# alexcoca/DistributedKernelShap

Measured on NVIDIA H100. Metric: instances explained/sec (bg=100, nsamples=2048) at 1/2/4/8 H100 vs ray CPU, higher is better.
Workload: dtype f32 sigmoid/accumulate, f64 link + WLS

## Files before the change

### distributedkernelshap_b200/csrc/dks.cu

```cuda
#include <algorithm>
#include <cmath>
#include <cstdarg>
#include <cstdio>
#include <cstring>
#include <memory>

#include "dks_kernels.cuh"
#include "dks_tc.cuh"
#include "dks_shared.cuh"
#include "dks_fused.cuh"
#include "dks_l1.cuh"
#include "dks_mixture.cuh"
#include "dks_multi.cuh"
#include "dks_wide.cuh"
#include "dks_sampler.cuh"
#include "dks_instance_wide.cuh"
#include "dks_trees.cuh"
#include "dks_encode.cuh"
#include "dks_kmach.cuh"
#include "dks_mlp.cuh"
#include "dks_knn.cuh"
#include "dks_ensemble.cuh"

namespace {
// ... 467 lines not shown
            m->own_X = ctx->own_X; m->own_D = ctx->own_D; m->own_bg = ctx->own_bg;
            m->own_goff = ctx->own_goff; m->own_gcols = ctx->own_gcols;
            const size_t msm = own_kernel(m->head.family).smem(m, p.S_cap);
            const dks::EnsAcc mea{ctx->d_ens_ey, ctx->h_ens_pi[k], k == 0 ? 1 : 0};
            TRY(on_member(ctx, m, [&] { return launch_own_kernel(m, false, p, msm, st, mea); }));
        }
        const size_t tsm = dks::ens::tail_smem_bytes(p.S_cap, ctx->C);
        auto kern = l1 ? dks::ens::explain_ensemble_tail_kernel<true> : dks::ens::explain_ensemble_tail_kernel<false>;
        CUDA_TRY(cudaFuncSetAttribute(kern, cudaFuncAttributeMaxDynamicSharedMemorySize, (int)tsm));
        kern<<<persistent_grid(ctx, tsm, 1024, 8, ctx->cur_n), dks::ens::THREADS, tsm, st>>>(p, q, ctx->d_ens_ey);
        break;
    }
    }
    ctx->launches += 1;
    return DKS_OK;
}

template <bool STAGE, bool MAPS>
decltype(&dks::prep_kernel<STAGE, MAPS>) prep_kernel_for(bool mixture, int R) {
    if (mixture) return dks::prep_kernel<STAGE, MAPS, true>;
    return R == 1 ? dks::prep_kernel<STAGE, MAPS, false, 1> : dks::prep_kernel<STAGE, MAPS, false, 8>;
}

int launch_prepare(dks_ctx* ctx, const double* X_dev, int n) {
    const int G = ctx->G;
    const HeadDesc& h = ctx->head;
    TRY(ensure_workspace(ctx, n));
    CUDA_TRY(cudaMemsetAsync(ctx->d_status, 0, sizeof(int) * (4 + G + 1), ctx->stream));
    if (!ctx->capturing) ctx->last_was_graph = false;
    CUDA_TRY(record_ev(ctx, 0));
    int ipb = 256 / G;
    if (ipb < 1) ipb = 1;
    const bool maps = ctx->cm.hdr != nullptr;
    const size_t maps_doubles = maps ? (size_t)ctx->cm.n_keys + ctx->cm.n_vals : 0;
    const bool stage = dks::prep_smem_bytes(true, ipb, G, ctx->R, ctx->D, maps_doubles) <= (size_t)96 * 1024;
    const size_t psm = dks::prep_smem_bytes(stage, ipb, G, ctx->R, ctx->D, maps_doubles);
    const bool own = h.own();
    const int R = own ? 1 : ctx->R;
    auto kern = stage ? (maps ? prep_kernel_for<true, true>(h.mixture(), R) : prep_kernel_for<true, false>(h.mixture(), R))
                      : (maps ? prep_kernel_for<false, true>(h.mixture(), R) : prep_kernel_for<false, false>(h.mixture(), R));
    double* xt = !own && (h.xt_any || (G <= 128 && ctx->plan_mode == 0)) ? ctx->d_XT.get() : nullptr;
    if (psm > 48 * 1024) CUDA_TRY(cudaFuncSetAttribute(kern, cudaFuncAttributeMaxDynamicSharedMemorySize, (int)psm));
    const bool enc = own && ctx->enc.E > 0;
    if (enc) TRY(grow(ctx, ctx->d_Xenc, (size_t)n * ctx->enc.E));
    ctx->own_X = enc ? ctx->d_Xenc : X_dev;
    ctx->own_D = enc ? ctx->enc.E : ctx->D;
    ctx->own_bg = enc ? ctx->d_bg_enc : ctx->d_bg;
    ctx->own_goff = enc ? ctx->d_egoff : ctx->d_goff;
    ctx->own_gcols = enc ? ctx->d_egcols : ctx->d_gcols;
    kern<<<cdiv(n, ipb), 256, psm, ctx->stream>>>(
        X_dev, ctx->d_W, ctx->d_b, ctx->d_bg, ctx->d_goff, ctx->d_gcols, ctx->d_colmin, ctx->d_colmax, ctx->d_colnan,
        ctx->d_linkfnull, n, ctx->N, ctx->D, G, R, own ? 1 : ctx->C, own ? DKS_ACT_IDENTITY : ctx->act, own ? 1.0 : ctx->kappa,
        ctx->link, ipb, ctx->d_XW, ctx->d_vmask, ctx->d_M, ctx->d_dlink, ctx->d_hist, ctx->d_counts, ctx->d_idx_full,
        ctx->d_idx_other, xt, h.xt_scale, h.xt_bbar ? ctx->d_Bbar.get() : nullptr, ctx->d_status, ctx->cm, ctx->d_mix);
    if (own) TRY(launch_own_predict(ctx, X_dev, n, enc ? ctx->d_Xenc.get() : nullptr, ctx->d_linkfnull, nullptr, ctx->d_dlink));
    ctx->launches += 1;
    CUDA_TRY(cudaGetLastError());
    CUDA_TRY(record_ev(ctx, 1));
    ctx->cur_n = n;
    ctx->cur_X = X_dev;
    ctx->prepared = true;
    return DKS_OK;
}

int launch_mix_axpy(dks_ctx* ctx, float* dst, float pi, bool first, int stride, int n) {
    long long grid = cdiv((long long)n * stride, 256);
    if (grid > (long long)ctx->sm_count * 8) grid = (long long)ctx->sm_count * 8;
    if (grid < 1) grid = 1;
    dks::mix::mix_axpy_kernel<<<(int)grid, 256, 0, ctx->stream>>>(ctx->d_mixscr, dst, pi, first ? 1 : 0, ctx->d_idx_full,
                                                                   ctx->d_counts, stride);
    ctx->launches += 1;
    CUDA_TRY(cudaGetLastError());
    return DKS_OK;
// ... 487 lines not shown
    ctx->gen_stride = sc.stride; ctx->gen_n = n; ctx->gen_plan_words = sc.W;
    p->ext_z = ctx->d_genz; p->ext_w = ctx->d_genw; p->ext_stride = sc.stride;
    p->ext_chol = rt.wide_pi ? nullptr : ctx->d_genchol.get(); p->ext_ainv = rt.wide_pi ? ctx->d_genchol : ctx->d_genainv;
    p->ext_fstride = sc.fstride;
    return DKS_OK;
}

int launch_shared_binary(dks_ctx* ctx, const Route& rt, const PlanDev& pg, double* phi_dev) {
    const int n = ctx->cur_n, G = ctx->G;
    int32_t* path = ctx->last_path;
    const float* wn = ctx->uniform_w ? nullptr : ctx->d_wn.get();
    if (rt.shared == ROUTE_FUSED) {
        const dks::shared_path::FusedConfig& fcfg = rt.fcfg;
        dks::shared_path::FusedParams fp;
        memset(&fp, 0, sizeof(fp));
        fp.n = n; fp.N = ctx->N; fp.G = G; fp.C = ctx->C; fp.S = pg.S; fp.S_pad = pg.S_pad; fp.link = ctx->link; fp.B = fcfg.B;
        fp.scale = ctx->head.scale; fp.DmT = pg.dmT; fp.dme = pg.dme; fp.z = pg.z; fp.XT = ctx->d_XT; fp.list = ctx->d_idx_full;
        fp.count = ctx->d_counts; fp.pmat64 = pg.pmat64; fp.dvec = pg.dvec64; fp.dlink = ctx->d_dlink;
        fp.linkfnull = ctx->d_linkfnull; fp.fnull = ctx->d_fnull; fp.acc = ctx->d_acc; fp.wn = wn;
        const bool table = ctx->opt_fused_table && pg.ltab != nullptr;
        if (table) {
            fp.ltab = pg.ltab; fp.ltab_rows = pg.ltab_rows; fp.ltab_inv_h = pg.ltab_inv_h; fp.ltab_fb = ctx->d_ltab_fb;
        }
        CUDA_TRY(dks::shared_path::launch_explain_fused(fp, fcfg, ctx->sm_count, ctx->stream));
        dks::PeerPush pp;
        pp.npeers = 0;
        if (ctx->peer_world > 1 && ctx->push_in_kernel) {
            for (int r = 0; r < ctx->peer_world; ++r) {
                double* slab = ctx->peer_base[r] + (long long)ctx->peer_rank * ctx->peer_slab;
                if (slab == phi_dev) continue;
                pp.dst[pp.npeers++] = slab;
            }
        }
        dks::shared_path::finish_fused_kernel<<<cdiv(n, 16), 256, 0, ctx->stream>>>(
            ctx->d_idx_full, ctx->d_counts, ctx->d_acc, dks::shared_path::fused_kpad(G), pg.dvec64, ctx->d_dlink, n, G, ctx->C,
            phi_dev, pp);
        ctx->launches += 1;
        path[DKS_PATH_SHARED] = DKS_SHARED_FUSED; path[DKS_PATH_CHUNKS] = 1; path[DKS_PATH_WARPS] = fcfg.warps;
        path[DKS_PATH_GRID] = ctx->sm_count; path[DKS_PATH_FUSED_B] = fcfg.B; path[DKS_PATH_FUSED_NI] = 1;
        path[DKS_PATH_SOLVE] = DKS_SOLVE_FUSED; path[DKS_PATH_FUSED_CTA_WARPS] = fcfg.slices * fcfg.kw;
        path[DKS_PATH_FUSED_TABLE] = table ? 1 : 0;
        CUDA_TRY(cudaGetLastError());
        return DKS_OK;
    }
    const size_t need = (size_t)n * pg.S_pad;
    TRY(grow(ctx, ctx->d_sums, need));
    dks::shared_path::SharedParams sp;
// ... 526 lines not shown
    cudaError_t e = cudaGetDeviceCount(&count);
    if (e != cudaSuccess || count == 0)
        return fail(DKS_ERR_CUDA, "dks_create: no CUDA device (%s) -- the engine has no CPU fallback",
                    cudaGetErrorString(e));
    if (device < 0 || device >= count) return fail(DKS_ERR_INVALID, "dks_create: device %d out of range [0,%d)", device, count);
    CUDA_TRY(cudaSetDevice(device));
    cudaDeviceProp prop;
    CUDA_TRY(cudaGetDeviceProperties(&prop, device));
    if (prop.major != 9 || prop.minor != 0)
        return fail(DKS_ERR_UNSUPPORTED, "dks_create: device %d is sm_%d%d; this library is built for sm_90a only", device,
                    prop.major, prop.minor);
    std::unique_ptr<dks_ctx> ctx(new dks_ctx());
    ctx->device = device;
    { const char* e = getenv("DKS_GRAPH"); ctx->graph_enabled = !(e && e[0] == '0'); }
    {
        auto env_int = [](const char* name, int dflt) { const char* e = getenv(name); return e ? atoi(e) : dflt; };
        ctx->opt_fused = env_int("DKS_FUSED", 1);
        ctx->opt_fused_warps = env_int("DKS_FUSED_WARPS", 0);
        ctx->opt_fused_B = env_int("DKS_FUSED_B", 0);
        ctx->push_in_kernel = env_int("DKS_PUSH_IN_KERNEL", 0) != 0;
    }
    ctx->sm_count = prop.multiProcessorCount;
    ctx->max_smem_optin = (int)prop.sharedMemPerBlockOptin;
    memset(ctx->h_plans, 0, sizeof(ctx->h_plans));
    CUDA_TRY(cudaStreamCreateWithFlags(&ctx->stream, cudaStreamNonBlocking));
    ctx->own_stream = true;
    for (int i = 0; i < 4; ++i) CUDA_TRY(cudaEventCreate(&ctx->ev[i]));
    for (int i = 0; i < 3; ++i) CUDA_TRY(cudaEventCreate(&ctx->ev_l1[i]));
    CUDA_TRY(cudaStreamCreateWithFlags(&ctx->side_stream, cudaStreamNonBlocking));
    CUDA_TRY(cudaEventCreateWithFlags(&ctx->ev_fork, cudaEventDisableTiming));
    CUDA_TRY(cudaEventCreateWithFlags(&ctx->ev_join, cudaEventDisableTiming));
    CUDA_TRY(ctx->d_plans.alloc(DKS_MAX_GROUPS + 1));
    CUDA_TRY(cudaMemset(ctx->d_plans, 0, sizeof(ctx->h_plans)));
    CUDA_TRY(ctx->status.alloc(4 + DKS_MAX_GROUPS + 1));
    ctx->d_status = ctx->status;
    ctx->d_counts = ctx->d_status + 2;
    ctx->d_hist = ctx->d_status + 4;
    CUDA_TRY(cudaMemset(ctx->d_status, 0, sizeof(int) * (4 + DKS_MAX_GROUPS + 1)));
    CUDA_TRY(ctx->d_l1.alloc(DKS_L1_MAX_GROUPS + 1));
    CUDA_TRY(cudaMemset(ctx->d_l1, 0, sizeof(dks::l1::Tables) * (DKS_L1_MAX_GROUPS + 1)));
    CUDA_TRY(ctx->d_l1_counts.alloc(2));
    *out = ctx.release();
    return DKS_OK;
}

int dks_destroy(dks_ctx* ctx) {
// ... 960 lines not shown
        CUDA_TRY(cudaGetLastError());
        return DKS_OK;
    }
    dim3 grid(8, pp.npeers);
    dks::push_phi_kernel<<<grid, 256, 0, ctx->stream>>>(phi_dev, pp, ctx->peer_slab);
    ctx->launches += 1;
    CUDA_TRY(cudaGetLastError());
    return DKS_OK;
}

static int launch_peer_sync(dks_ctx* ctx) {
    if (ctx->peer_world <= 1 || !ctx->peer_flags_set) return DKS_OK;
    dks::PeerFlags f;
    memset(&f, 0, sizeof(f));
    f.world = ctx->peer_world; f.rank = ctx->peer_rank; f.step = ctx->d_step;
    f.mine = ctx->peer_flags[ctx->peer_rank];
    for (int r = 0; r < ctx->peer_world; ++r) f.peer[r] = ctx->peer_flags[r];
    dks::peer_sync_kernel<<<1, 32, 0, ctx->stream>>>(f, ctx->d_status);
    ctx->launches += 1;
    CUDA_TRY(cudaGetLastError());
    return DKS_OK;
}

static void drop_graph(dks_ctx* ctx) {
    if (ctx->gexec) { cudaGraphExecDestroy(ctx->gexec); ctx->gexec = nullptr; }
}

int dks_run_dev(dks_ctx* ctx, const double* X_dev, int n, double* phi_dev) {
    BIND(ctx);
    REQUIRE(ctx->fitted, "dks_run_dev: call dks_fit first");
    REQUIRE(X_dev && phi_dev && n > 0, "dks_run_dev: bad arguments");
    dks_ctx::GraphKey key{X_dev, phi_dev, n, ctx->nsamples_req, ctx->kernel_choice, ctx->plan_mode, ctx->row_offset,
                          (unsigned long long)ctx->sampler_seed, ctx->epoch, ctx->stream};
    if (ctx->graph_enabled && ctx->gexec && key == ctx->graph_key && ctx->dbg_i < 0) {
        CUDA_TRY(cudaGraphLaunch(ctx->gexec, ctx->stream));
        ctx->graph_launches++;
        ctx->launches += ctx->graph_kernels;
        ctx->last_was_graph = true;
        return DKS_OK;
    }
    const bool capturable = ctx->stream != nullptr && ctx->stream != cudaStreamLegacy && ctx->stream != cudaStreamPerThread;
    bool capture = ctx->graph_enabled && capturable && ctx->have_last_key && key == ctx->last_key && ctx->dbg_i < 0;
    ctx->last_key = key; ctx->have_last_key = true;
    if (capture) {
        drop_graph(ctx);
        if (cudaStreamBeginCapture(ctx->stream, cudaStreamCaptureModeRelaxed) != cudaSuccess) {
            cudaGetLastError();
            ctx->graph_enabled = false;
            capture = false;
        } else {
            ctx->capturing = true;
        }
    }
    const int64_t launches_before = ctx->launches;
    int rc = launch_prepare(ctx, X_dev, n);
    if (rc == DKS_OK) rc = launch_explain(ctx, phi_dev, nullptr, nullptr, 0);
    if (rc == DKS_OK) rc = launch_push(ctx, phi_dev);
    if (rc == DKS_OK) rc = launch_peer_sync(ctx);
    ctx->last_was_graph = capture;
    if (capture) {
        ctx->capturing = false;
        cudaGraph_t graph = nullptr;
        cudaError_t ce = cudaStreamEndCapture(ctx->stream, &graph);
        if (rc == DKS_OK && ce == cudaSuccess && graph) {
            ce = cudaGraphInstantiate(&ctx->gexec, graph, 0);
            if (ce == cudaSuccess) {
                ctx->graph_key = key;
                ctx->graph_kernels = ctx->launches - launches_before;
                ce = cudaGraphLaunch(ctx->gexec, ctx->stream);
                ctx->graph_launches++;
            }
        }
        if (graph) cudaGraphDestroy(graph);
        if (rc != DKS_OK) return rc;
        if (ce != cudaSuccess) {
            drop_graph(ctx);
            cudaGetLastError();
            ctx->graph_enabled = false;
            ctx->launches = launches_before;
            TRY(launch_prepare(ctx, X_dev, n));
            TRY(launch_explain(ctx, phi_dev, nullptr, nullptr, 0));
            TRY(launch_push(ctx, phi_dev));
            TRY(launch_peer_sync(ctx));
        }
    } else if (rc != DKS_OK) {
        return rc;
    }
    return DKS_OK;
}

int dks_set_peers(dks_ctx* ctx, int world, int rank, const uint64_t* gathered_ptrs_host, int64_t slab_doubles) {
    REQUIRE(ctx, "dks_set_peers: ctx is NULL");
    ctx->epoch++;
    if (world <= 1 || gathered_ptrs_host == nullptr) { ctx->peer_world = 0; ctx->peer_flags_set = false; return DKS_OK; }
    REQUIRE(world <= 16 && rank >= 0 && rank < world && slab_doubles > 0, "dks_set_peers: bad arguments (at most 16 ranks)");
    for (int r = 0; r < world; ++r) {
        REQUIRE(gathered_ptrs_host[r] != 0 && (gathered_ptrs_host[r] & 15) == 0, "dks_set_peers: peer buffers must be 16-byte aligned");
        ctx->peer_base[r] = reinterpret_cast<double*>(gathered_ptrs_host[r]);
    }
    REQUIRE((slab_doubles & 1) == 0, "dks_set_peers: slab size must be even (128-bit stores)");
    ctx->peer_world = world; ctx->peer_rank = rank; ctx->peer_slab = slab_doubles;
    return DKS_OK;
}
// ... 219 lines not shown
```

### distributedkernelshap_b200/csrc/dks_common.cuh

```cuda
#pragma once

#include <cuda_runtime.h>
#include <stdint.h>

#include <atomic>
#include <string>
#include <utility>
#include <vector>

#include "dks.h"

namespace dks {
inline std::atomic<int64_t> g_live_allocations{0};

inline cudaError_t mem_alloc(void** p, size_t bytes, bool pinned) {
    const cudaError_t e = pinned ? cudaHostAlloc(p, bytes, cudaHostAllocDefault) : cudaMalloc(p, bytes);
    if (e == cudaSuccess) g_live_allocations++;
    return e;
}

inline void mem_free(void* p, bool pinned) {
    if (!p) return;
    if (pinned) cudaFreeHost(p);
    else cudaFree(p);
// ... 280 lines not shown
    const float* lo[DKS_MIX_MAX_R];
    const double* ell;
};

__device__ __forceinline__ int dks_inst_count(const ExplainParams& p) { return p.list ? *p.count : p.n; }
__device__ __forceinline__ int dks_inst_at(const ExplainParams& p, int q) { return p.list ? p.list[q] : q; }

struct dks_ctx {
    ~dks_ctx() {
        if (gexec) cudaGraphExecDestroy(gexec);
        for (cudaEvent_t e : ev) if (e) cudaEventDestroy(e);
        for (cudaEvent_t e : ev_l1) if (e) cudaEventDestroy(e);
        if (ev_fork) cudaEventDestroy(ev_fork);
        if (ev_join) cudaEventDestroy(ev_join);
        if (side_stream) cudaStreamDestroy(side_stream);
        if (own_stream && stream) cudaStreamDestroy(stream);
    }

    int device = 0;
    cudaStream_t stream = nullptr;
    bool own_stream = false;
    int sm_count = 132;
    int max_smem_optin = 0;

    int N = 0, D = 0, G = 0, R = 0, C = 0;
    int act = -1, link = DKS_LINK_IDENTITY, scalar_out = 0;
    double kappa = 1.0;
    bool fitted = false;
    int kernel_choice = DKS_KERNEL_AUTO;
    int nsamples_req = 0;
    bool uniform_w = true;
    DevBuf<float> dbg_T;
    int dbg_i = -1, dbg_rows = 0, dbg_cols = 0;
    DevBuf<float> dbg_time;

    MixHead mix = {};
    DevBuf<MixHead> d_mix;
    DevBuf<double> d_mixBW;
    DevBuf<double> d_mixsc;
    DevBuf<float> d_mixscr;
    std::vector<int32_t> h_tfeat, h_tleft, h_tright, h_troots;
    std::vector<double> h_tthr, h_tval, h_tbase;
    std::vector<unsigned char> h_tmiss;
    TreeDev tree = {};
    DevBuf<unsigned char> txinfo;
    std::vector<int32_t> h_ehdr, h_eops;
// ... 135 lines not shown
```

### distributedkernelshap_b200/csrc/dks_fused.cuh

```cuda
#pragma once

#include "dks_shared.cuh"

namespace dks {
namespace shared_path {

constexpr double LTAB_MARGIN = 33.0;
constexpr double LTAB_TOL = 1e-9;
constexpr size_t LTAB_BUDGET = (size_t)256 << 20;
constexpr int LTAB_NODES = 6;

struct __align__(16) LinkTabEntry { double c0, c1; float c2, c3, c4, c5; };
struct __align__(16) LinkTabRow { double x_lo; int off, nint; };
static_assert(sizeof(LinkTabEntry) == 32, "one interval is 32 bytes");

struct LinkTabFit { double t[LTAB_NODES]; double vinv[LTAB_NODES * LTAB_NODES]; };

__host__ __device__ __forceinline__ double ltab_poly(const LinkTabEntry& e, double t) {
    const float tf = (float)t;
    const float q = fmaf(tf, fmaf(tf, fmaf(tf, e.c5, e.c4), e.c3), e.c2);
    return fma(t, fma(t, (double)q, e.c1), e.c0);
}

__device__ double ltab_exact(double x, const double* __restrict__ ld, int S_pad, const double* __restrict__ wd, int N, int link) {
// ... 149 lines not shown
    const int nq = dm_quads(NCT ? NCT : p.N);
    const int nqw = dm_quads_w(NCT ? NCT : p.N);
    const int sq4 = WT ? 2 * nqw : nq;
    const int nsl = flat ? 2 : slices;
    float4* sDm = reinterpret_cast<float4*>(fsm);
    double* sP = reinterpret_cast<double*>(sDm + (size_t)nsl * sq4 * 32);
    double* sY = sP + (size_t)nsl * 32 * KPAD;
    LogTabEntry* s_logtab = reinterpret_cast<LogTabEntry*>(sY + (size_t)slices * kw * 32 * ystride);
    float2* sW2 = reinterpret_cast<float2*>(s_logtab + DKS_LOGTAB_SIZE);
    if (threadIdx.x >= 64 && threadIdx.x < 64 + DKS_LOGTAB_SIZE) logtab_fill(s_logtab, threadIdx.x - 64);
    if constexpr (WT) {
        for (int q = threadIdx.x; q < nqw; q += blockDim.x) sW2[q] = w2_quad(p.wn, NCT ? NCT : p.N, q);
    }

    constexpr int MAXCH = MAXN / 16;
    const int N = NCT ? NCT : p.N;
    const int nfull = N / 16, ntail = N - nfull * 16;
    const int nch = nfull + (ntail > 0 ? 1 : 0);
    const int n_rg = p.S_pad / 32;
    const int nparts = gridDim.x * slices / n_rg;
    const int gs = blockIdx.x * slices + slice;
    const bool active = slice < slices && (flat || gs < nparts * n_rg);
    double* sYw = sY + (size_t)warp * 32 * ystride;
    const int cnt_f = flat ? *p.count : 0;
    const long long U = (long long)n_rg * cnt_f;
    const long long c0 = U * blockIdx.x / gridDim.x, c1 = U * (blockIdx.x + 1) / gridDim.x;
    const long long u0 = c0 + (c1 - c0) * sub / kw, u1 = c0 + (c1 - c0) * (sub + 1) / kw;
    const int rg_lo = cnt_f > 0 ? (int)(c0 / cnt_f) : 0;
    const int nfill = flat ? (c1 > c0 ? (int)((c1 - 1) / cnt_f) - rg_lo + 1 : 0) : 1;
    for (int f = 0; active && f < nfill; ++f) {
        const int fs = flat ? f : slice;
        const int rg = flat ? rg_lo + f : gs % n_rg;
        const int s = rg * 32 + lane;
        double* sPw = sP + (size_t)fs * 32 * KPAD;
        float4* sl = sDm + (size_t)fs * sq4 * 32;
        const double* src = p.pmat64 + (size_t)rg * 32 * KPAD;
        for (int idx = sub * 32 + lane; idx < 32 * KPAD; idx += 32 * kw) sPw[idx] = src[idx];
        if constexpr (WT) {
            for (int q = sub; q < nqw; q += kw) {
                float4 sq, xy;
                dm_quad_w(p.DmT, p.wn, N, p.S_pad, s, q, sq, xy);
                sl[(2 * q) * 32 + lane] = sq;
                sl[(2 * q + 1) * 32 + lane] = xy;
            }
        }
#pragma unroll
        for (int c = 0; c < MAXCH; ++c) {
            if (!WT && c < nch && c % kw == sub) {
                float v[16];
#pragma unroll
                for (int jj = 0; jj < 16; ++jj) {
                    const int j = c * 16 + jj;
                    v[jj] = j < N ? p.DmT[(size_t)j * p.S_pad + s] : 0.f;
                }
                const int nv = c < nfull ? 16 : ntail;
#pragma unroll
                for (int jj = 0; jj < 16; jj += 4) {
                    if (jj + 3 < nv) {
                        const float d0 = v[jj], d1 = v[jj + 1], d2 = v[jj + 2], d3 = v[jj + 3];
                        v[jj] = d0 + d2; v[jj + 1] = d1 + d3; v[jj + 2] = d0 * d2; v[jj + 3] = d1 * d3;
                    }
                }
                dm_st16(sl, c, nq, lane, v);
            }
        }
    }
    __syncthreads();

    if (active) {
        const int cnt = *p.count;
        const int G = p.G, nA = G - 1;
        const int nq_t = ntail >> 2, rem_t = ntail & 3;
        const long long seg_end = flat && u0 < u1 ? ((u0 / cnt) + 1) * cnt : 0;
        const int nseg = flat ? (u0 < u1 ? (u1 > seg_end ? 2 : 1) : 0) : 1;
        const int rg0 = flat ? (u0 < u1 ? (int)(u0 / cnt) : 0) : gs % n_rg;
        const int first0 = flat ? (u0 < u1 ? (int)(u0 % cnt) : 0) : gs / n_rg + sub * nparts;
        const int my_n0 = flat ? (int)((u1 < seg_end ? u1 : seg_end) - u0) : 0, my_n1 = flat ? (int)(u1 - seg_end) : 0;
        for (int seg = 0; seg < nseg; ++seg) {
            const int rg = rg0 + seg;
            const int s = rg * 32 + lane;
            const int fs = flat ? rg - rg_lo : slice;
            const double* sPw = sP + (size_t)fs * 32 * KPAD;
            const float4* sl = sDm + (size_t)fs * sq4 * 32;
            const int first = seg == 0 ? first0 : 0;
            const int stride = flat ? 1 : nparts * kw;
            const int my_n = flat ? (seg == 0 ? my_n0 : my_n1) : (first < cnt ? (cnt - first + stride - 1) / stride : 0);
            const double es = p.dme[s];
            const uint64_t zz = s < p.S ? p.z[s] : 0ull;
            const int ntab = (G + 3) / 4;
            const f32x2 one2 = f2_pack(1.f, 1.f), two2 = f2_pack(2.f, 2.f);
            const double yf = p.link == DKS_LINK_LOGIT ? p.linkfnull[1] : p.fnull[1], inv_n = 1.0 / (double)N;
            const bool row_ok = s < p.S;
            const int bmask = B - 1;
// ... 252 lines not shown
    const int n_rg = S_pad / 32;
    if ((long long)sm_count * warps < n_rg) return false;
    auto flat_fits = [&](int R, int K) {
        return R == 1 && fused_flat_smem_bytes(K, kpad, B, N, weighted) + 1024 <= (size_t)max_smem;
    };
    auto busy = [&](int R, int K) {
        if (K > 1 && flat_fits(R, K)) return (long long)K * sm_count;
        return (long long)K * ((long long)sm_count * R / n_rg) * n_rg;
    };
    const int max_cta = fused_max_cta_warps(N, kpad, weighted);
    const int cap = want_warps > 0 && want_warps < max_cta ? want_warps : max_cta;
    int slices = warps, kw = 1;
    for (int R = 1; R <= warps && cap / R >= 2; ++R) {
        const int K = cap / R;
        if ((long long)sm_count * R < n_rg || fused_smem_bytes(R, K, kpad, B, N, weighted) + 1024 > (size_t)max_smem) continue;
        if (busy(R, K) > busy(slices, kw)) { slices = R; kw = K; }
    }
    cfg->warps = warps; cfg->slices = slices; cfg->kw = kw; cfg->B = B;
    cfg->flat = kw > 1 && flat_fits(slices, kw) ? 1 : 0;
    cfg->smem = cfg->flat ? fused_flat_smem_bytes(kw, kpad, B, N, weighted) : fused_smem_bytes(slices, kw, kpad, B, N, weighted);
    return true;
}

inline cudaError_t launch_explain_fused(const FusedParams& p, const FusedConfig& cfg, int grid, cudaStream_t stream) {
    const int kpad = fused_kpad(p.G);
    cudaError_t err = cudaSuccess;
#define DKS_FUSED_LAUNCH(NCT, KP, NW)                                                                                 \
    do {                                                                                                              \
        err = cudaFuncSetAttribute(explain_shared_fused_kernel<NCT, KP, NW>, cudaFuncAttributeMaxDynamicSharedMemorySize, \
                                   (int)cfg.smem);                                                                    \
        if (err == cudaSuccess)                                                                                       \
            explain_shared_fused_kernel<NCT, KP, NW><<<grid, 32 * NW, cfg.smem, stream>>>(p, cfg.slices, cfg.kw, cfg.flat); \
    } while (0)
    const int cta_warps = cfg.slices * cfg.kw;
    if (p.wn != nullptr) {
#define DKS_FUSED_LAUNCH_WT(NCT, KP, NW)                                                                              \
    do {                                                                                                              \
        err = cudaFuncSetAttribute(explain_shared_fused_kernel<NCT, KP, NW, true>,                                 \
                                   cudaFuncAttributeMaxDynamicSharedMemorySize, (int)cfg.smem);                       \
        if (err == cudaSuccess)                                                                                       \
            explain_shared_fused_kernel<NCT, KP, NW, true><<<grid, 32 * NW, cfg.smem, stream>>>(p, cfg.slices, cfg.kw, cfg.flat); \
    } while (0)
#define DKS_FUSED_WT(NCT, KP)                                                                                         \
    do {                                                                                                              \
        if (cta_warps > 16) DKS_FUSED_LAUNCH_WT(NCT, KP, 20);                                                         \
        else if (cta_warps > 12) DKS_FUSED_LAUNCH_WT(NCT, KP, 16);                                                    \
        else DKS_FUSED_LAUNCH_WT(NCT, KP, 12);                                                                        \
    } while (0)
#define DKS_FUSED_WT16(NCT, KP)                                                                                       \
    do {                                                                                                              \
        if (cta_warps > 12) DKS_FUSED_LAUNCH_WT(NCT, KP, 16);                                                         \
        else DKS_FUSED_LAUNCH_WT(NCT, KP, 12);                                                                        \
    } while (0)
        if (kpad == 12) {
            if (p.N == 100) DKS_FUSED_WT(100, 12);
            else if (p.N == 128) DKS_FUSED_WT(128, 12);
            else DKS_FUSED_WT16(0, 12);
        } else {
            if (p.N == 100) DKS_FUSED_WT(100, 16);
            else if (p.N == 128) DKS_FUSED_WT(128, 16);
            else DKS_FUSED_WT16(0, 16);
        }
#undef DKS_FUSED_WT16
#undef DKS_FUSED_WT
#undef DKS_FUSED_LAUNCH_WT
// ... 26 lines not shown
```

### distributedkernelshap_b200/csrc/dks_kernels.cuh

```cuda
#pragma once

#include <cuda_pipeline.h>

#include "dks_common.cuh"
#include "dks_linkmath.cuh"

namespace dks {

__device__ __forceinline__ float ex2_approx(float x) {
    float y;
    asm("ex2.approx.ftz.f32 %0, %1;" : "=f"(y) : "f"(x));
    return y;
}
__device__ __forceinline__ float rcp_approx(float x) {
    float y;
    asm("rcp.approx.ftz.f32 %0, %1;" : "=f"(y) : "f"(x));
    return y;
}
__device__ __forceinline__ double warp_sum(double v) {
#pragma unroll
    for (int o = 16; o > 0; o >>= 1) v += __shfl_xor_sync(0xffffffffu, v, o);
    return v;
}

// ... 239 lines not shown
                            const double* __restrict__ bg, const int32_t* __restrict__ goff,
                            const int32_t* __restrict__ gcols, const double* __restrict__ colmin,
                            const double* __restrict__ colmax, const int* __restrict__ colnan,
                            const double* __restrict__ linkfnull, int n, int N, int D, int G, int R, int C, int act,
                            double kappa, int link, int ipb, double* __restrict__ XW, uint64_t* __restrict__ vmask,
                            int* __restrict__ Mcnt, double* __restrict__ dlink, int* __restrict__ hist,
                            int* __restrict__ counts, int* __restrict__ idx_full, int* __restrict__ idx_other,
                            double* __restrict__ XT, double xt_scale, const double* __restrict__ xt_sub,
                            int* __restrict__ status, ColumnMapsDev cm, const MixHead* __restrict__ mix) {
    constexpr int CB = MIX ? 8 : (RB == 1 ? 2 : RB);
    extern __shared__ __align__(16) unsigned char prep_smem[];
    double* sXW = reinterpret_cast<double*>(prep_smem);
    double* sX = sXW + (size_t)ipb * G * R;
    double* sW = sX + (STAGE ? (size_t)ipb * D : 0);
    double* sMin = sW + (STAGE ? (MAPS ? (size_t)cm.n_keys + cm.n_vals : (size_t)R * D) : 0);
    double* sMax = sMin + (STAGE ? D : 0);
    int* sNan = reinterpret_cast<int*>(sMax + (STAGE ? D : 0));
    int* sCols = sNan + (STAGE ? D : 0);
    int* sOff = sCols + (STAGE ? D : 0);
    int* sHdr = sOff + (STAGE ? G + 1 : 0);
    int* sCnt = sHdr + (STAGE && MAPS ? 4 * D : 0);
    int* sHist = sCnt + 4;
    unsigned char* sflag = reinterpret_cast<unsigned char*>(sHist + G + 1);
    for (int idx = threadIdx.x; idx < G + 5; idx += blockDim.x) sCnt[idx] = 0;
    if (threadIdx.x == 0) {
        asm volatile("prefetch.global.L2 [%0];" ::"l"(b));
        asm volatile("prefetch.global.L2 [%0];" ::"l"(linkfnull));
    }
    const int i0 = blockIdx.x * ipb;
    if (STAGE) {
        auto cp8 = [](double* d, const double* s) { __pipeline_memcpy_async(d, s, sizeof(double)); };
        auto cp4 = [](int* d, const int* s) { __pipeline_memcpy_async(d, s, sizeof(int)); };
        const int rows = min(ipb, n - i0);
        const double* Xb = X + (size_t)i0 * D;
        for (int idx = threadIdx.x; idx < rows * D; idx += blockDim.x) cp8(sX + idx, Xb + idx);
        if (MAPS) {
            for (int idx = threadIdx.x; idx < cm.n_keys; idx += blockDim.x) cp8(sW + idx, cm.keys + idx);
            for (int idx = threadIdx.x; idx < cm.n_vals; idx += blockDim.x) cp8(sW + cm.n_keys + idx, cm.vals + idx);
            for (int idx = threadIdx.x; idx < 4 * D; idx += blockDim.x) cp4(sHdr + idx, cm.hdr + idx);
        } else {
            for (int idx = threadIdx.x; idx < R * D; idx += blockDim.x) cp8(sW + idx, W + idx);
        }
        for (int idx = threadIdx.x; idx < D; idx += blockDim.x) {
            cp8(sMin + idx, colmin + idx); cp8(sMax + idx, colmax + idx);
            cp4(sNan + idx, colnan + idx); cp4(sCols + idx, gcols + idx);
        }
// ... 19 lines not shown
                    cm_report(status, i);
            } else {
#pragma unroll
                for (int r = 0; r < RB; ++r)
                    if (r < R) acc[r] += xv * (STAGE ? sW[(size_t)r * D + col] : W[(size_t)r * D + col]);
            }
            if ((STAGE ? sNan[col] : colnan[col]) || isnan(xv)) {
                if (!varies)
                    for (int j = 0; j < N && !varies; ++j) varies = !np_isclose(xv, bg[(size_t)j * D + col]);
            } else {
                const double mn = STAGE ? sMin[col] : colmin[col], mx = STAGE ? sMax[col] : colmax[col];
                varies = varies || !np_isclose(xv, mn) || !np_isclose(xv, mx);
            }
        }
#pragma unroll
        for (int r = 0; r < RB; ++r) {
            if (r >= R) continue;
            sXW[(size_t)idx * R + r] = acc[r];
            XW[((size_t)i * G + g) * R + r] = acc[r];
        }
        sflag[idx] = varies ? 1 : 0;
    }
    __syncthreads();
    if (XT != nullptr) {
        const int ntab = (G + 3) / 4;
        for (int idx = threadIdx.x; idx < ipb * R * ntab * 16; idx += blockDim.x) {
            const int li = idx / (R * ntab * 16), rem = idx - li * R * ntab * 16, r = rem / (ntab * 16);
            const int t = (rem >> 4) - r * ntab, x = rem & 15;
            const int i = i0 + li;
            if (i >= n) continue;
            double acc = 0.0;
#pragma unroll
            for (int b = 0; b < 4; ++b)
                if (((x >> b) & 1) && 4 * t + b < G) {
                    const int k = 4 * t + b;
                    acc += xt_sub != nullptr ? sXW[((size_t)li * G + k) * R + r] - xt_sub[(size_t)k * R + r]
                                             : sXW[((size_t)li * G + k) * R + r];
                }
            const size_t row = MIX ? ((size_t)(r / mix->Rm) * n + i) * mix->Rm + r % mix->Rm : (size_t)i * R + r;
            XT[(row * ntab + t) * 16 + x] = xt_scale * acc;
        }
    }
    const int li = threadIdx.x, i = i0 + li;
    const bool mine = li < ipb && i < n;
    int list = 0, rank = 0;
    if (mine) {
        uint64_t m = 0;
        int M = 0;
        double z[RB], o[CB];
#pragma unroll
        for (int r = 0; r < RB; ++r) z[r] = r < R ? b[r] : 0.0;
        for (int g = 0; g < G; ++g) {
            if (sflag[li * G + g]) { if (g < 64) m |= (1ull << g); ++M; }
#pragma unroll
            for (int r = 0; r < RB; ++r) if (r < R) z[r] += sXW[((size_t)li * G + g) * R + r];
        }
        vmask[i] = m;
        Mcnt[i] = M;
        atomicAdd(&sHist[M], 1);
        list = M == G && M >= 2 ? 0 : 1;
        rank = atomicAdd(&sCnt[list], 1);
        if constexpr (MIX) mix_head_f64(z, *mix, o);
        else head_f64<RB>(z, R, act, kappa, o);
#pragma unroll
        for (int c = 0; c < CB; ++c)
            if (c < C) dlink[(size_t)i * C + c] = link_f(o[c], link) - linkfnull[c];
        if (act == DKS_ACT_EXP && !isfinite(o[0]) && atomicCAS(&status[0], 0, DKS_ERR_NUMERIC) == 0) status[1] = i;
    }
    __syncthreads();
    if (threadIdx.x < 2 && sCnt[threadIdx.x] > 0) sCnt[2 + threadIdx.x] = atomicAdd(&counts[threadIdx.x], sCnt[threadIdx.x]);
    for (int t = threadIdx.x; t <= G; t += blockDim.x)
        if (sHist[t] > 0) atomicAdd(&hist[t], sHist[t]);
    __syncthreads();
    if (mine) (list == 0 ? idx_full : idx_other)[sCnt[2 + list] + rank] = i;
}
inline size_t prep_smem_bytes(bool stage, int ipb, int G, int R, int D, size_t maps_doubles = 0) {
    size_t b = sizeof(double) * (size_t)ipb * G * R + sizeof(int) * ((size_t)G + 5) + (size_t)ipb * G + 16;
    if (stage && maps_doubles)
        b += sizeof(double) * ((size_t)ipb * D + maps_doubles + 2 * (size_t)D) + sizeof(int) * (6 * (size_t)D + G + 1);
    else if (stage)
        b += sizeof(double) * ((size_t)ipb * D + (size_t)R * D + 2 * (size_t)D) + sizeof(int) * (2 * (size_t)D + G + 1);
    return b;
}


__device__ inline void wls_build_normal(const uint64_t* __restrict__ zp, const double* __restrict__ wp, int S, int M,
                                        double* A, int warp, int nwarps) {
    const int nA = M - 1, L = M - 1;
    const int lane = threadIdx.x & 31;
    const int npairs = nA * (nA + 1) / 2;
    for (int pr = warp; pr < npairs; pr += nwarps) {
        int k = 0, rem = pr;
        while (rem > k) { rem -= (k + 1); ++k; }
        int l = rem;
        double acc = 0;
        for (int s = lane; s < S; s += 32) {
            uint64_t z = zp[s];
// ... 687 lines not shown
```

### distributedkernelshap_b200/engine.py

```python
import ctypes as C
import logging

import numpy as np

from . import _cabi
from .data import DenseData, convert_to_data, convert_to_link
from .ensembles import MAX_GROUPS as ENSEMBLE_MAX_GROUPS, EnsembleSpec, extract_ensemble_spec
from .plan import build_plan, l1_tables, pack_dense_plan, projection, resolve_nsamples, sampling_info
from .kernel_machines import MAX_GROUPS as KMACH_MAX_GROUPS, KernelMachineSpec, extract_kernel_machine_spec
from .mlp import MAX_GROUPS as MLP_MAX_GROUPS, MlpSpec, extract_mlp_spec
from .neighbors import MAX_GROUPS as KNN_MAX_GROUPS, KnnSpec, extract_knn_spec
from .predictors import extract_linear_spec
from .trees import MAX_GROUPS as TREE_MAX_GROUPS, TreeEnsembleSpec, extract_encoded_pipeline_spec, \
    extract_tree_pipeline_spec, extract_tree_spec

logger = logging.getLogger(__name__)

MODEL_CHECK_RTOL = 1e-9
MAX_ROWS_PER_CALL = 65536
MAX_ROWS_PER_CALL_WIDE_PER_INSTANCE = 4096
MAX_SAMPLED_SIZES = 64
MAX_ENCODED_BYTES_PER_CALL = 256 << 20
MAX_ENSEMBLE_BYTES_PER_CALL = 1 << 30

# ... 625 lines not shown
        out = np.zeros(3, dtype=np.float32)
        _cabi.check(self.lib.dks_last_timings(self._ctx, _cabi.ptr(out)))
        return {"prepare": float(out[0]), "coalitions": float(out[1]), "total": float(out[2])}

    _PATH_NAMES = {
        "shared": ("none", "fused", "smem", None, "softmax", "affine", "ovr", "exp", "mixture"),
        "solve": ("none", "fused", "pmat", "wls_shared", "wide", "l1"),
        "general": ("none", "tc", "simt", "flagged", "simt_wide", "trees", "kmach", "mlp", "knn", "ensemble"),
    }

    def last_path(self):
        out = np.zeros(13, dtype=np.int32)
        _cabi.check(self.lib.dks_last_path(self._ctx, _cabi.ptr(out), len(out)))
        names = self._PATH_NAMES
        general = names["general"][out[8]]
        if out[12] and self._l1_general_all_select:
            general = "simt"
        return {"shared": names["shared"][out[0]], "chunks": int(out[1]), "warps": int(out[2]), "grid": int(out[3]),
                "fused_B": int(out[4]), "fused_NI": int(out[5]), "solve": names["solve"][out[6]],
                "pmat_kpad": int(out[7]), "general": general,
                "cta_warps": int(out[9]), "bg_weights": ("uniform", "weighted")[out[10]], "fused_table": int(out[11]),
                "general_l1": int(out[12])}

    def general_l1_timings_ms(self):
        out = np.zeros(2, dtype=np.float32)
        _cabi.check(self.lib.dks_last_general_l1_timings(self._ctx, _cabi.ptr(out)))
        return {"general": float(out[0]), "lars": float(out[1])}

    def fused_table_info(self, M):
        nbytes, fb = C.c_int64(0), C.c_int64(0)
        _cabi.check(self.lib.dks_fused_table_info(self._ctx, int(M), C.byref(nbytes), C.byref(fb)))
        return {"bytes": int(nbytes.value), "fallback_passes": int(fb.value)}

    def debug_scores(self, X, instance, nsamples="auto"):
        _cabi.check(self.lib.dks_debug_score_dump(self._ctx, int(instance)))
        try:
            self.shap_values(X, nsamples=nsamples, l1_reg=False)
            buf = np.zeros(1 << 22, dtype=np.float32)
            rows, cols = C.c_int(0), C.c_int(0)
            _cabi.check(self.lib.dks_debug_get_scores(self._ctx, _cabi.ptr(buf), buf.size, C.byref(rows), C.byref(cols)))
        finally:
            _cabi.check(self.lib.dks_debug_score_dump(self._ctx, -1))
        return buf[:rows.value * cols.value].reshape(rows.value, cols.value).copy()

    def debug_timeline(self, X, nsamples="auto"):
        self.shap_values(X, nsamples=nsamples, l1_reg=False)
# ... 20 lines not shown
```

### include/dks.h

```cpp
#ifndef DKS_H_
#define DKS_H_

#include <stdint.h>

#ifdef __cplusplus
extern "C" {
#endif

#define DKS_VERSION 100

#define DKS_OK 0
#define DKS_ERR_INVALID 1
#define DKS_ERR_CUDA 2
#define DKS_ERR_UNSUPPORTED 3
#define DKS_ERR_PLAN_MISSING 4
#define DKS_ERR_NUMERIC 5
#define DKS_ERR_DOMAIN 6

#define DKS_ACT_IDENTITY 0
#define DKS_ACT_BINARY_LOGISTIC 1
#define DKS_ACT_SOFTMAX 2
#define DKS_ACT_OVR 3
#define DKS_ACT_EXP 4
#define DKS_ACT_MIX 5
// ... 143 lines not shown
int dks_last_status(dks_ctx* ctx, int* detail);

int dks_summarise_host(dks_ctx* ctx, int n, const int32_t* seg_offsets_host, int Gp, double* phi_sum_host,
                       double* mean_abs_host, int32_t* order_host, int32_t* argmax_host);

int dks_set_kernel(dks_ctx* ctx, int kernel);
int dks_set_option(dks_ctx* ctx, const char* name, int value);
int dks_kernel_launches(dks_ctx* ctx, int64_t* count);
int dks_live_allocations(int64_t* count);
int dks_fused_table_info(dks_ctx* ctx, int M, int64_t* table_bytes, int64_t* fallback_passes);
#define DKS_PATH_SHARED 0
#define DKS_PATH_CHUNKS 1
#define DKS_PATH_WARPS 2
#define DKS_PATH_GRID 3
#define DKS_PATH_FUSED_B 4
#define DKS_PATH_FUSED_NI 5
#define DKS_PATH_SOLVE 6
#define DKS_PATH_PMAT_KPAD 7
#define DKS_PATH_GENERAL 8
#define DKS_PATH_FUSED_CTA_WARPS 9
#define DKS_PATH_BG_WEIGHTS 10
#define DKS_PATH_FUSED_TABLE 11
#define DKS_PATH_GENERAL_L1 12
#define DKS_PATH_FIELDS 13
#define DKS_SHARED_NONE 0
#define DKS_SHARED_FUSED 1
#define DKS_SHARED_SMEM 2
#define DKS_SHARED_SOFTMAX 4
#define DKS_SHARED_AFFINE 5
#define DKS_SHARED_OVR 6
#define DKS_SHARED_EXP 7
#define DKS_SHARED_MIX 8
#define DKS_SOLVE_NONE 0
#define DKS_SOLVE_FUSED 1
#define DKS_SOLVE_PMAT 2
#define DKS_SOLVE_WLS_SHARED 3
#define DKS_SOLVE_WIDE 4
#define DKS_SOLVE_L1 5
#define DKS_GENERAL_NONE 0
#define DKS_GENERAL_TC 1
#define DKS_GENERAL_SIMT 2
#define DKS_GENERAL_FLAGGED 3
#define DKS_GENERAL_SIMT_WIDE 4
#define DKS_GENERAL_TREES 5
#define DKS_GENERAL_KMACH 6
#define DKS_GENERAL_MLP 7
#define DKS_GENERAL_KNN 8
// ... 14 lines not shown
```

Measured before the change: 38.82 million.

## Overlap prep and fused explain kernels via programmatic dependent launch

Launches the fused explain kernel with programmatic stream serialization. The prep kernel triggers launch_dependents early and the fused kernel runs its background/table staging before griddepcontrol.wait, so fused setup overlaps prep execution. Prep is reordered to publish counts before the XT fill, its block size is cut to 128 on the fused route, the status memset becomes a tiny kernel so it can sit in the graph, and an shared-memory carveout is set so prep and fused CTAs can co-reside on an SM. The fused kernel's flat work split now derives fill ranges from n instead of the device count, which is read only after the wait. This risks subtle ordering bugs if any pre-wait work depends on prep outputs, and the smaller prep blocks may reduce prep throughput.

```diff
diff --git a/distributedkernelshap_b200/csrc/dks.cu b/distributedkernelshap_b200/csrc/dks.cu
--- a/distributedkernelshap_b200/csrc/dks.cu
+++ b/distributedkernelshap_b200/csrc/dks.cu
@@ -513,14 +513,13 @@
     return R == 1 ? dks::prep_kernel<STAGE, MAPS, false, 1> : dks::prep_kernel<STAGE, MAPS, false, 8>;
 }
 
-int launch_prepare(dks_ctx* ctx, const double* X_dev, int n) {
+int launch_prepare(dks_ctx* ctx, const double* X_dev, int n, const dks::shared_path::FusedConfig* fused = nullptr) {
     const int G = ctx->G;
     const HeadDesc& h = ctx->head;
     TRY(ensure_workspace(ctx, n));
-    CUDA_TRY(cudaMemsetAsync(ctx->d_status, 0, sizeof(int) * (4 + G + 1), ctx->stream));
     if (!ctx->capturing) ctx->last_was_graph = false;
-    CUDA_TRY(record_ev(ctx, 0));
-    int ipb = 256 / G;
+    const int threads = fused ? 128 : 256;
+    int ipb = threads / G;
     if (ipb < 1) ipb = 1;
     const bool maps = ctx->cm.hdr != nullptr;
     const size_t maps_doubles = maps ? (size_t)ctx->cm.n_keys + ctx->cm.n_vals : 0;
@@ -532,6 +531,9 @@
                       : (maps ? prep_kernel_for<false, true>(h.mixture(), R) : prep_kernel_for<false, false>(h.mixture(), R));
     double* xt = !own && (h.xt_any || (G <= 128 && ctx->plan_mode == 0)) ? ctx->d_XT.get() : nullptr;
     if (psm > 48 * 1024) CUDA_TRY(cudaFuncSetAttribute(kern, cudaFuncAttributeMaxDynamicSharedMemorySize, (int)psm));
+    ctx->step_carveout = fused ? dks::shared_path::fused_carveout(fused->smem, psm, ctx->smem_per_sm)
+                               : (int)cudaSharedmemCarveoutDefault;
+    CUDA_TRY(cudaFuncSetAttribute(kern, cudaFuncAttributePreferredSharedMemoryCarveout, ctx->step_carveout));
     const bool enc = own && ctx->enc.E > 0;
     if (enc) TRY(grow(ctx, ctx->d_Xenc, (size_t)n * ctx->enc.E));
     ctx->own_X = enc ? ctx->d_Xenc : X_dev;
@@ -539,7 +541,10 @@
     ctx->own_bg = enc ? ctx->d_bg_enc : ctx->d_bg;
     ctx->own_goff = enc ? ctx->d_egoff : ctx->d_goff;
     ctx->own_gcols = enc ? ctx->d_egcols : ctx->d_gcols;
-    kern<<<cdiv(n, ipb), 256, psm, ctx->stream>>>(
+    CUDA_TRY(cudaFuncSetAttribute(dks::clear_step_kernel, cudaFuncAttributePreferredSharedMemoryCarveout, ctx->step_carveout));
+    dks::clear_step_kernel<<<1, 256, 0, ctx->stream>>>(ctx->d_status, 4 + G + 1);
+    CUDA_TRY(record_ev(ctx, 0));
+    kern<<<cdiv(n, ipb), threads, psm, ctx->stream>>>(
         X_dev, ctx->d_W, ctx->d_b, ctx->d_bg, ctx->d_goff, ctx->d_gcols, ctx->d_colmin, ctx->d_colmax, ctx->d_colnan,
         ctx->d_linkfnull, n, ctx->N, ctx->D, G, R, own ? 1 : ctx->C, own ? DKS_ACT_IDENTITY : ctx->act, own ? 1.0 : ctx->kappa,
         ctx->link, ipb, ctx->d_XW, ctx->d_vmask, ctx->d_M, ctx->d_dlink, ctx->d_hist, ctx->d_counts, ctx->d_idx_full,
@@ -1073,7 +1078,7 @@
         if (table) {
             fp.ltab = pg.ltab; fp.ltab_rows = pg.ltab_rows; fp.ltab_inv_h = pg.ltab_inv_h; fp.ltab_fb = ctx->d_ltab_fb;
         }
-        CUDA_TRY(dks::shared_path::launch_explain_fused(fp, fcfg, ctx->sm_count, ctx->stream));
+        CUDA_TRY(dks::shared_path::launch_explain_fused(fp, fcfg, ctx->sm_count, ctx->step_carveout, ctx->stream));
         dks::PeerPush pp;
         pp.npeers = 0;
         if (ctx->peer_world > 1 && ctx->push_in_kernel) {
@@ -1646,6 +1651,7 @@
     }
     ctx->sm_count = prop.multiProcessorCount;
     ctx->max_smem_optin = (int)prop.sharedMemPerBlockOptin;
+    ctx->smem_per_sm = (int)prop.sharedMemPerMultiprocessor;
     memset(ctx->h_plans, 0, sizeof(ctx->h_plans));
     CUDA_TRY(cudaStreamCreateWithFlags(&ctx->stream, cudaStreamNonBlocking));
     ctx->own_stream = true;
@@ -2652,6 +2658,21 @@
     return DKS_OK;
 }
 
+static cudaError_t count_programmatic_edges(cudaGraph_t graph, int32_t* count) {
+    *count = 0;
+    std::vector<cudaGraphNode_t> from(64), to(64);
+    std::vector<cudaGraphEdgeData> data(64);
+    size_t ne = from.size();
+    cudaError_t err = cudaGraphGetEdges_v2(graph, from.data(), to.data(), data.data(), &ne);
+    if (err == cudaSuccess && ne > from.size()) {
+        from.resize(ne); to.resize(ne); data.resize(ne);
+        err = cudaGraphGetEdges_v2(graph, from.data(), to.data(), data.data(), &ne);
+    }
+    for (size_t e = 0; err == cudaSuccess && e < ne; ++e)
+        if (data[e].type == cudaGraphDependencyTypeProgrammatic) ++*count;
+    return err;
+}
+
 static void drop_graph(dks_ctx* ctx) {
     if (ctx->gexec) { cudaGraphExecDestroy(ctx->gexec); ctx->gexec = nullptr; }
 }
@@ -2683,7 +2704,9 @@
         }
     }
     const int64_t launches_before = ctx->launches;
-    int rc = launch_prepare(ctx, X_dev, n);
+    Route rt;
+    const bool fused = choose_route(ctx, nullptr, 0, &rt) == DKS_OK && rt.shared == ROUTE_FUSED;
+    int rc = launch_prepare(ctx, X_dev, n, fused ? &rt.fcfg : nullptr);
     if (rc == DKS_OK) rc = launch_explain(ctx, phi_dev, nullptr, nullptr, 0);
     if (rc == DKS_OK) rc = launch_push(ctx, phi_dev);
     if (rc == DKS_OK) rc = launch_peer_sync(ctx);
@@ -2693,7 +2716,8 @@
         cudaGraph_t graph = nullptr;
         cudaError_t ce = cudaStreamEndCapture(ctx->stream, &graph);
         if (rc == DKS_OK && ce == cudaSuccess && graph) {
-            ce = cudaGraphInstantiate(&ctx->gexec, graph, 0);
+            ce = count_programmatic_edges(graph, &ctx->last_path[DKS_PATH_GRAPH_PDL_EDGES]);
+            if (ce == cudaSuccess) ce = cudaGraphInstantiate(&ctx->gexec, graph, 0);
             if (ce == cudaSuccess) {
                 ctx->graph_key = key;
                 ctx->graph_kernels = ctx->launches - launches_before;
@@ -2708,7 +2732,7 @@
             cudaGetLastError();
             ctx->graph_enabled = false;
             ctx->launches = launches_before;
-            TRY(launch_prepare(ctx, X_dev, n));
+            TRY(launch_prepare(ctx, X_dev, n, fused ? &rt.fcfg : nullptr));
             TRY(launch_explain(ctx, phi_dev, nullptr, nullptr, 0));
             TRY(launch_push(ctx, phi_dev));
             TRY(launch_peer_sync(ctx));
diff --git a/distributedkernelshap_b200/csrc/dks_common.cuh b/distributedkernelshap_b200/csrc/dks_common.cuh
--- a/distributedkernelshap_b200/csrc/dks_common.cuh
+++ b/distributedkernelshap_b200/csrc/dks_common.cuh
@@ -326,6 +326,8 @@
     bool own_stream = false;
     int sm_count = 132;
     int max_smem_optin = 0;
+    int smem_per_sm = 0;
+    int step_carveout = -1;
 
     int N = 0, D = 0, G = 0, R = 0, C = 0;
     int act = -1, link = DKS_LINK_IDENTITY, scalar_out = 0;
diff --git a/distributedkernelshap_b200/csrc/dks_fused.cuh b/distributedkernelshap_b200/csrc/dks_fused.cuh
--- a/distributedkernelshap_b200/csrc/dks_fused.cuh
+++ b/distributedkernelshap_b200/csrc/dks_fused.cuh
@@ -195,12 +195,13 @@
     const int gs = blockIdx.x * slices + slice;
     const bool active = slice < slices && (flat || gs < nparts * n_rg);
     double* sYw = sY + (size_t)warp * 32 * ystride;
-    const int cnt_f = flat ? *p.count : 0;
-    const long long U = (long long)n_rg * cnt_f;
-    const long long c0 = U * blockIdx.x / gridDim.x, c1 = U * (blockIdx.x + 1) / gridDim.x;
-    const long long u0 = c0 + (c1 - c0) * sub / kw, u1 = c0 + (c1 - c0) * (sub + 1) / kw;
-    const int rg_lo = cnt_f > 0 ? (int)(c0 / cnt_f) : 0;
-    const int nfill = flat ? (c1 > c0 ? (int)((c1 - 1) / cnt_f) - rg_lo + 1 : 0) : 1;
+    const int rg_lo = flat ? (int)((long long)n_rg * blockIdx.x / gridDim.x) : 0;
+    int nfill = 1;
+    if (flat) {
+        const long long U = (long long)n_rg * p.n;
+        const long long c0 = U * blockIdx.x / gridDim.x, c1 = U * (blockIdx.x + 1) / gridDim.x;
+        nfill = c1 > c0 ? (int)((c1 - 1) / p.n) - rg_lo + 1 : 0;
+    }
     for (int f = 0; active && f < nfill; ++f) {
         const int fs = flat ? f : slice;
         const int rg = flat ? rg_lo + f : gs % n_rg;
@@ -238,10 +239,14 @@
             }
         }
     }
+    asm volatile("griddepcontrol.wait;" ::: "memory");
     __syncthreads();
 
     if (active) {
         const int cnt = *p.count;
+        const long long U = flat ? (long long)n_rg * cnt : 0;
+        const long long c0 = U * blockIdx.x / gridDim.x, c1 = U * (blockIdx.x + 1) / gridDim.x;
+        const long long u0 = c0 + (c1 - c0) * sub / kw, u1 = c0 + (c1 - c0) * (sub + 1) / kw;
         const int G = p.G, nA = G - 1;
         const int nq_t = ntail >> 2, rem_t = ntail & 3;
         const long long seg_end = flat && u0 < u1 ? ((u0 / cnt) + 1) * cnt : 0;
@@ -540,25 +545,37 @@
     return true;
 }
 
-inline cudaError_t launch_explain_fused(const FusedParams& p, const FusedConfig& cfg, int grid, cudaStream_t stream) {
+inline int fused_carveout(size_t fused_smem, size_t prep_smem, int smem_per_sm) {
+    const size_t need = fused_smem + prep_smem + 2048;
+    const size_t pct = (100 * need + (size_t)smem_per_sm - 1) / (size_t)smem_per_sm;
+    return pct < 100 ? (int)pct : 100;
+}
+
+template <typename Kernel>
+inline cudaError_t launch_fused_dependent(Kernel kern, const FusedParams& p, const FusedConfig& cfg, int grid, int threads,
+                                          int carveout, cudaStream_t stream) {
+    cudaError_t err = cudaFuncSetAttribute(kern, cudaFuncAttributeMaxDynamicSharedMemorySize, (int)cfg.smem);
+    if (err == cudaSuccess) err = cudaFuncSetAttribute(kern, cudaFuncAttributePreferredSharedMemoryCarveout, carveout);
+    if (err != cudaSuccess) return err;
+    cudaLaunchAttribute attr[1];
+    attr[0].id = cudaLaunchAttributeProgrammaticStreamSerialization;
+    attr[0].val.programmaticStreamSerializationAllowed = 1;
+    cudaLaunchConfig_t lc = {};
+    lc.gridDim = dim3(grid); lc.blockDim = dim3(threads); lc.dynamicSmemBytes = cfg.smem; lc.stream = stream;
+    lc.attrs = attr; lc.numAttrs = 1;
+    return cudaLaunchKernelEx(&lc, kern, p, cfg.slices, cfg.kw, cfg.flat);
+}
+
+inline cudaError_t launch_explain_fused(const FusedParams& p, const FusedConfig& cfg, int grid, int carveout,
+                                        cudaStream_t stream) {
     const int kpad = fused_kpad(p.G);
     cudaError_t err = cudaSuccess;
-#define DKS_FUSED_LAUNCH(NCT, KP, NW)                                                                                 \
-    do {                                                                                                              \
-        err = cudaFuncSetAttribute(explain_shared_fused_kernel<NCT, KP, NW>, cudaFuncAttributeMaxDynamicSharedMemorySize, \
-                                   (int)cfg.smem);                                                                    \
-        if (err == cudaSuccess)                                                                                       \
-            explain_shared_fused_kernel<NCT, KP, NW><<<grid, 32 * NW, cfg.smem, stream>>>(p, cfg.slices, cfg.kw, cfg.flat); \
-    } while (0)
+#define DKS_FUSED_LAUNCH(NCT, KP, NW) \
+    err = launch_fused_dependent(explain_shared_fused_kernel<NCT, KP, NW>, p, cfg, grid, 32 * NW, carveout, stream)
     const int cta_warps = cfg.slices * cfg.kw;
     if (p.wn != nullptr) {
-#define DKS_FUSED_LAUNCH_WT(NCT, KP, NW)                                                                              \
-    do {                                                                                                              \
-        err = cudaFuncSetAttribute(explain_shared_fused_kernel<NCT, KP, NW, true>,                                 \
-                                   cudaFuncAttributeMaxDynamicSharedMemorySize, (int)cfg.smem);                       \
-        if (err == cudaSuccess)                                                                                       \
-            explain_shared_fused_kernel<NCT, KP, NW, true><<<grid, 32 * NW, cfg.smem, stream>>>(p, cfg.slices, cfg.kw, cfg.flat); \
-    } while (0)
+#define DKS_FUSED_LAUNCH_WT(NCT, KP, NW) \
+    err = launch_fused_dependent(explain_shared_fused_kernel<NCT, KP, NW, true>, p, cfg, grid, 32 * NW, carveout, stream)
 #define DKS_FUSED_WT(NCT, KP)                                                                                         \
     do {                                                                                                              \
         if (cta_warps > 16) DKS_FUSED_LAUNCH_WT(NCT, KP, 20);                                                         \
diff --git a/distributedkernelshap_b200/csrc/dks_kernels.cuh b/distributedkernelshap_b200/csrc/dks_kernels.cuh
--- a/distributedkernelshap_b200/csrc/dks_kernels.cuh
+++ b/distributedkernelshap_b200/csrc/dks_kernels.cuh
@@ -285,6 +285,7 @@
     int* sCnt = sHdr + (STAGE && MAPS ? 4 * D : 0);
     int* sHist = sCnt + 4;
     unsigned char* sflag = reinterpret_cast<unsigned char*>(sHist + G + 1);
+    asm volatile("griddepcontrol.launch_dependents;");
     for (int idx = threadIdx.x; idx < G + 5; idx += blockDim.x) sCnt[idx] = 0;
     if (threadIdx.x == 0) {
         asm volatile("prefetch.global.L2 [%0];" ::"l"(b));
@@ -350,6 +351,36 @@
         sflag[idx] = varies ? 1 : 0;
     }
     __syncthreads();
+    const int li = threadIdx.x, i = i0 + li;
+    const bool mine = li < ipb && i < n;
+    int list = 0, rank = 0;
+    if (mine) {
+        uint64_t m = 0;
+        int M = 0;
+        double z[RB], o[CB];
+#pragma unroll
+        for (int r = 0; r < RB; ++r) z[r] = r < R ? b[r] : 0.0;
+        for (int g = 0; g < G; ++g) {
+            if (sflag[li * G + g]) { if (g < 64) m |= (1ull << g); ++M; }
+#pragma unroll
+            for (int r = 0; r < RB; ++r) if (r < R) z[r] += sXW[((size_t)li * G + g) * R + r];
+        }
+        vmask[i] = m;
+        Mcnt[i] = M;
+        atomicAdd(&sHist[M], 1);
+        list = M == G && M >= 2 ? 0 : 1;
+        rank = atomicAdd(&sCnt[list], 1);
+        if constexpr (MIX) mix_head_f64(z, *mix, o);
+        else head_f64<RB>(z, R, act, kappa, o);
+#pragma unroll
+        for (int c = 0; c < CB; ++c)
+            if (c < C) dlink[(size_t)i * C + c] = link_f(o[c], link) - linkfnull[c];
+        if (act == DKS_ACT_EXP && !isfinite(o[0]) && atomicCAS(&status[0], 0, DKS_ERR_NUMERIC) == 0) status[1] = i;
+    }
+    __syncthreads();
+    if (threadIdx.x < 2 && sCnt[threadIdx.x] > 0) sCnt[2 + threadIdx.x] = atomicAdd(&counts[threadIdx.x], sCnt[threadIdx.x]);
+    for (int t = threadIdx.x; t <= G; t += blockDim.x)
+        if (sHist[t] > 0) atomicAdd(&hist[t], sHist[t]);
     if (XT != nullptr) {
         const int ntab = (G + 3) / 4;
         for (int idx = threadIdx.x; idx < ipb * R * ntab * 16; idx += blockDim.x) {
@@ -369,38 +400,11 @@
             XT[(row * ntab + t) * 16 + x] = xt_scale * acc;
         }
     }
-    const int li = threadIdx.x, i = i0 + li;
-    const bool mine = li < ipb && i < n;
-    int list = 0, rank = 0;
-    if (mine) {
-        uint64_t m = 0;
-        int M = 0;
-        double z[RB], o[CB];
-#pragma unroll
-        for (int r = 0; r < RB; ++r) z[r] = r < R ? b[r] : 0.0;
-        for (int g = 0; g < G; ++g) {
-            if (sflag[li * G + g]) { if (g < 64) m |= (1ull << g); ++M; }
-#pragma unroll
-            for (int r = 0; r < RB; ++r) if (r < R) z[r] += sXW[((size_t)li * G + g) * R + r];
-        }
-        vmask[i] = m;
-        Mcnt[i] = M;
-        atomicAdd(&sHist[M], 1);
-        list = M == G && M >= 2 ? 0 : 1;
-        rank = atomicAdd(&sCnt[list], 1);
-        if constexpr (MIX) mix_head_f64(z, *mix, o);
-        else head_f64<RB>(z, R, act, kappa, o);
-#pragma unroll
-        for (int c = 0; c < CB; ++c)
-            if (c < C) dlink[(size_t)i * C + c] = link_f(o[c], link) - linkfnull[c];
-        if (act == DKS_ACT_EXP && !isfinite(o[0]) && atomicCAS(&status[0], 0, DKS_ERR_NUMERIC) == 0) status[1] = i;
-    }
-    __syncthreads();
-    if (threadIdx.x < 2 && sCnt[threadIdx.x] > 0) sCnt[2 + threadIdx.x] = atomicAdd(&counts[threadIdx.x], sCnt[threadIdx.x]);
-    for (int t = threadIdx.x; t <= G; t += blockDim.x)
-        if (sHist[t] > 0) atomicAdd(&hist[t], sHist[t]);
     __syncthreads();
     if (mine) (list == 0 ? idx_full : idx_other)[sCnt[2 + list] + rank] = i;
+}
+__global__ void clear_step_kernel(int* __restrict__ w, int count) {
+    for (int k = threadIdx.x; k < count; k += blockDim.x) w[k] = 0;
 }
 inline size_t prep_smem_bytes(bool stage, int ipb, int G, int R, int D, size_t maps_doubles = 0) {
     size_t b = sizeof(double) * (size_t)ipb * G * R + sizeof(int) * ((size_t)G + 5) + (size_t)ipb * G + 16;
diff --git a/distributedkernelshap_b200/engine.py b/distributedkernelshap_b200/engine.py
--- a/distributedkernelshap_b200/engine.py
+++ b/distributedkernelshap_b200/engine.py
@@ -671,6 +671,11 @@
                 "cta_warps": int(out[9]), "bg_weights": ("uniform", "weighted")[out[10]], "fused_table": int(out[11]),
                 "general_l1": int(out[12])}
 
+    def graph_programmatic_edges(self):
+        out = np.zeros(14, dtype=np.int32)
+        _cabi.check(self.lib.dks_last_path(self._ctx, _cabi.ptr(out), len(out)))
+        return int(out[13])
+
     def general_l1_timings_ms(self):
         out = np.zeros(2, dtype=np.float32)
         _cabi.check(self.lib.dks_last_general_l1_timings(self._ctx, _cabi.ptr(out)))
diff --git a/include/dks.h b/include/dks.h
--- a/include/dks.h
+++ b/include/dks.h
@@ -189,7 +189,8 @@
 #define DKS_PATH_BG_WEIGHTS 10
 #define DKS_PATH_FUSED_TABLE 11
 #define DKS_PATH_GENERAL_L1 12
-#define DKS_PATH_FIELDS 13
+#define DKS_PATH_GRAPH_PDL_EDGES 13
+#define DKS_PATH_FIELDS 14
 #define DKS_SHARED_NONE 0
 #define DKS_SHARED_FUSED 1
 #define DKS_SHARED_SMEM 2
```

Result: faster. 39.82 million, median of 6 (+2.6%).
